# swesterfeld/audiowmark

Measured on AMD Instinct MI355X. Metric: audio seconds watermarked+decoded per wall-second (xRT), 44.1 kHz stereo, higher is better.
Workload: dtype f32; 1 GPU; 60 min stereo 44.1 kHz white noise per GPU resident in HBM, add+get incl. payload decode, payload 0123456789abcdef0011223344556677, strength 10; parallelism=1 GPU, patterns=108, payload_matches=104, ranks_seen=1

## Files before the change

### audiowmark_amd/csrc/hip/viterbi.hip

```cpp
#include "kernels.hh"
#include <atomic>
#include <chrono>
#include <cstdio>
#include <mutex>
#include <type_traits>
#include <utility>

namespace awmk {

namespace {

constexpr int V_ORDER = 15;
constexpr int V_STATES = 1 << V_ORDER;
constexpr int V_WG = 256;

__device__ constexpr unsigned V_GEN_AB[12] = { 066561, 075211, 071545, 054435, 063635, 052475, 063543, 075307, 052547, 045627, 067657, 051757 };

template<int BT> __device__ constexpr unsigned v_gen (int g) { return BT == 2 ? V_GEN_AB[g] : V_GEN_AB[2 * g + BT]; }
__device__ constexpr unsigned v_parity (unsigned v) { v ^= v >> 16; v ^= v >> 8; v ^= v >> 4; v ^= v >> 2; v ^= v >> 1; return v & 1; }

typedef float v2f __attribute__ ((ext_vector_type (2)));

__device__ __forceinline__ v2f
pk_add_sel (v2f d, v2f pair, bool a, bool b)
// ... 240 lines not shown
  float *m_out = reinterpret_cast<float *> (ws + (parity_in ? 0 : V_METRIC_BYTES));
  unsigned int *dec = reinterpret_cast<unsigned int *> (ws + 2 * V_METRIC_BYTES) + dec_offset;
  const float *coded = b.soft[t] + (size_t) blk * b.n_steps * rate;
  const bool finite = *block_flag (ws, b.block_ws_bytes) == 0;
  if (t == 0)
    {
      if (PLAIN && finite) viterbi_round<0, K, true> (coded, step0, m_in, m_out, dec, L);
      else                 viterbi_round<0, K, false> (coded, step0, m_in, m_out, dec, L);
    }
  else if (t == 1)
    {
      if (PLAIN && finite) viterbi_round<1, K, true> (coded, step0, m_in, m_out, dec, L);
      else                 viterbi_round<1, K, false> (coded, step0, m_in, m_out, dec, L);
    }
  else
    {
      if (PLAIN && finite) viterbi_round<2, K, true> (coded, step0, m_in, m_out, dec, L);
      else                 viterbi_round<2, K, false> (coded, step0, m_in, m_out, dec, L);
    }
}

constexpr int SUPER_LDS = 16 * 324;

template<int BT, int NPF, bool COH = false> __device__ __forceinline__ void
viterbi_super_round (const float *coded, int step0, const float *m_in, float *m_out, unsigned int *dec, const size_t (&dec_off)[3],
                     int g, int lane, float *lds_a, float *lds_b, bool in_perm, bool out_perm, bool first = false)
{
  float m[16];
  const int L1 = (lane << 3) | g;
#pragma unroll
  for (int j = 0; j < 16; j++)
    m[j] = first ? ((L1 | j) == 0 ? 0.f : -1.f)
                 : ld_metric<COH> (in_perm ? m_in + g * 4096 + ((j << 8) | lane) : m_in + L1 + j * 2048);
  const int hi = lane >> 4, lo = lane & 15;
#pragma unroll
  for (int r = 0; r < 3; r++)
    {
      const int L = r == 0 ? L1 : r == 1 ? ((hi << 7) | (g << 4) | lo) : ((g << 8) | lane);
      unsigned int words[4];
      if (r < NPF)
        viterbi_steps<BT, 4, false> (coded, step0 + 4 * r, m, words, L);
      else
        viterbi_steps<BT, 4, true> (coded, step0 + 4 * r, m, words, L);
      st_words<COH> (dec + dec_off[r] + (size_t) L * 4, words[0], words[1], words[2], words[3]);
      if (r < 2)
        {
          float *x = r == 0 ? lds_a : lds_b;
#pragma unroll
          for (int loc = 0; loc < 16; loc++)
            x[loc * 324 + lo * 20 + hi] = m[loc];
          __syncthreads();
          const float4 *src = reinterpret_cast<const float4 *> (x + lo * 324 + hi * 20);
#pragma unroll
          for (int q = 0; q < 4; q++)
            {
              const float4 v = src[q];
              m[4 * q] = v.x; m[4 * q + 1] = v.y; m[4 * q + 2] = v.z; m[4 * q + 3] = v.w;
            }
        }
    }
  if (out_perm)
    {
#pragma unroll
      for (int f = 0; f < 8; f++)
        st_pair<COH> (m_out + f * 4096 + (g << 9) + (lane << 1), m[f], m[f + 8]);
      return;
    }
  float *out = m_out + (size_t) ((g << 8) | lane) * 16;
#pragma unroll
  for (int q = 0; q < 4; q++)
    st_quad<COH> (out + 4 * q, m[4 * q], m[4 * q + 1], m[4 * q + 2], m[4 * q + 3]);
}

struct SuperOffsets { size_t off[3]; int in_perm, out_perm, first; };

template<int NPF> __global__ void __launch_bounds__ (V_WG)
viterbi_super_kernel (ViterbiBatch b, int step0, int parity_in, SuperOffsets so)
{
  __shared__ float lds_a[SUPER_LDS], lds_b[SUPER_LDS];
  int blk = blockIdx.y, t = 0;
  if (blk >= b.n[0]) { blk -= b.n[0]; t = 1; }
  if (t == 1 && blk >= b.n[1]) { blk -= b.n[1]; t = 2; }
  const int rate = t == 2 ? 12 : 6;
  const int g = blockIdx.x, lane = threadIdx.x;
  unsigned char *ws = b.ws[t] + (size_t) blk * b.block_ws_bytes;
  const float *m_in = reinterpret_cast<const float *> (ws + (parity_in ? V_METRIC_BYTES : 0));
  float *m_out = reinterpret_cast<float *> (ws + (parity_in ? 0 : V_METRIC_BYTES));
  unsigned int *dec = reinterpret_cast<unsigned int *> (ws + 2 * V_METRIC_BYTES);
  const float *coded = b.soft[t] + (size_t) blk * b.n_steps * rate;
  if (so.first && g == 0)
    {
      const bool has_nan = block_has_nan (coded, b.n_steps * rate);
      if (lane == 0)
        *block_flag (ws, b.block_ws_bytes) = has_nan;
    }
  const bool finite = so.first || *block_flag (ws, b.block_ws_bytes) == 0;
  if (t == 0)
    {
      if (finite) viterbi_super_round<0, NPF> (coded, step0, m_in, m_out, dec, so.off, g, lane, lds_a, lds_b, so.in_perm != 0, so.out_perm != 0, so.first != 0);
      else        viterbi_super_round<0, 3> (coded, step0, m_in, m_out, dec, so.off, g, lane, lds_a, lds_b, so.in_perm != 0, so.out_perm != 0, so.first != 0);
    }
  else if (t == 1)
    {
      if (finite) viterbi_super_round<1, NPF> (coded, step0, m_in, m_out, dec, so.off, g, lane, lds_a, lds_b, so.in_perm != 0, so.out_perm != 0, so.first != 0);
      else        viterbi_super_round<1, 3> (coded, step0, m_in, m_out, dec, so.off, g, lane, lds_a, lds_b, so.in_perm != 0, so.out_perm != 0, so.first != 0);
    }
  else
    {
      if (finite) viterbi_super_round<2, NPF> (coded, step0, m_in, m_out, dec, so.off, g, lane, lds_a, lds_b, so.in_perm != 0, so.out_perm != 0, so.first != 0);
      else        viterbi_super_round<2, 3> (coded, step0, m_in, m_out, dec, so.off, g, lane, lds_a, lds_b, so.in_perm != 0, so.out_perm != 0, so.first != 0);
    }
}

__global__ void __launch_bounds__ (256)
viterbi_init_kernel (ViterbiBatch b)
{
  int blk = blockIdx.y, t = 0;
  if (blk >= b.n[0]) { blk -= b.n[0]; t = 1; }
  if (t == 1 && blk >= b.n[1]) { blk -= b.n[1]; t = 2; }
  unsigned char *ws = b.ws[t] + (size_t) blk * b.block_ws_bytes;
  float *m = reinterpret_cast<float *> (ws);
  const int i = blockIdx.x * 256 + threadIdx.x;
  m[i] = i == 0 ? 0.f : -1.f;
  if (blockIdx.x == 0)
    {
      const int rate = t == 2 ? 12 : 6;
      const bool has_nan = block_has_nan (b.soft[t] + (size_t) blk * b.n_steps * rate, b.n_steps * rate);
      if (threadIdx.x == 0)
        *block_flag (ws, b.block_ws_bytes) = has_nan;
    }
}

constexpr int MAX_ROUNDS = 64;
struct TracePlan
// ... 17 lines not shown
      const int K = plan.k[r];
      const unsigned L = state >> K;
      unsigned loc = state & ((1u << K) - 1);
      const int DW = dec_words (K);
      unsigned int w[5] = { 0, 0, 0, 0, 0 };
      const unsigned int *p = dec + plan.dec_offset[r] + (size_t) L * DW;
      const uint4 a = ld_words<COH> (p);
      w[0] = a.x; w[1] = a.y; w[2] = a.z; w[3] = a.w;
      if (DW == 8)
        w[4] = ld_words<COH> (p + 4).x;
      for (int i = K; i >= 1; i--)
        {
          const int step = plan.step0[r] + i - 1;
          if (step < n_steps - V_ORDER)
            bits[step] = loc & 1;
          const unsigned choose_high = (w[i - 1] >> loc) & 1;
          loc = (loc >> 1) | (choose_high << (K - 1));
        }
      state = L + (loc << (V_ORDER - K));
    }
}

template<bool COH> __device__ __forceinline__ void
viterbi_trace_wave (const TracePlan& plan, int final_parity, const unsigned char *ws, int n_steps, int rate, int *bits, float *error, int lane)
{
  const float *metric = reinterpret_cast<const float *> (ws + (final_parity ? V_METRIC_BYTES : 0));
  const unsigned int *dec = reinterpret_cast<const unsigned int *> (ws + 2 * V_METRIC_BYTES);
  if (lane == 0)
    *error = ld_metric<COH> (metric) / float (n_steps * rate);
  const int n_out = n_steps - V_ORDER;
  auto walk = [&] (const unsigned int (&w)[4], int K, unsigned loc, int step0) -> unsigned {
#pragma unroll
    for (int i = 4; i >= 1; i--)
      if (i <= K)
        {
          const int step = step0 + i - 1;
          if (step < n_out && lane == 0)
            bits[step] = loc & 1;
          const unsigned choose_high = (w[i - 1] >> loc) & 1;
          loc = (loc >> 1) | (choose_high << (K - 1));
        }
    return loc;
  };
  auto pick = [] (const uint4& v, unsigned from_lane, unsigned int (&w)[4]) {
    w[0] = __builtin_amdgcn_readlane (v.x, from_lane);
    w[1] = __builtin_amdgcn_readlane (v.y, from_lane);
    w[2] = __builtin_amdgcn_readlane (v.z, from_lane);
    w[3] = __builtin_amdgcn_readlane (v.w, from_lane);
  };
  unsigned state = 0;
  int r = plan.n_rounds - 1;
  while (r >= 0)
    {
      const int K = plan.k[r];
      if (r >= 2 && K == 4 && plan.k[r - 1] == 4 && plan.k[r - 2] == 4)
        {
          const unsigned L0 = state >> 4;
          const uint4 a = ld_words<COH> (dec + plan.dec_offset[r] + (size_t) L0 * 4);
          const unsigned c1 = lane & 15;
          const uint4 b1 = ld_words<COH> (dec + plan.dec_offset[r - 1] + (size_t) ((L0 >> 4) | (c1 << 7)) * 4);
          uint4 c2[4];
#pragma unroll
          for (int q = 0; q < 4; q++)
            {
              const unsigned idx = lane + 64 * q, c = idx & 15, e = idx >> 4;
              c2[q] = ld_words<COH> (dec + plan.dec_offset[r - 2] + (size_t) ((L0 >> 8) | (c << 3) | (e << 7)) * 4);
            }
          unsigned int w[4];
          pick (a, 0, w);
          const unsigned la = __builtin_amdgcn_readfirstlane (walk (w, 4, state & 15, plan.step0[r]));
          const unsigned s1 = L0 | (la << 11);
          pick (b1, la, w);
          const unsigned lb = __builtin_amdgcn_readfirstlane (walk (w, 4, s1 & 15, plan.step0[r - 1]));
// ... 18 lines not shown
      const unsigned L = state >> K;
      const uint4 a = ld_words<COH> (dec + plan.dec_offset[r] + (size_t) L * dec_words (K));
      unsigned int w[4];
      pick (a, 0, w);
      const unsigned l = __builtin_amdgcn_readfirstlane (walk (w, K, state & ((1u << K) - 1), plan.step0[r]));
      state = L | (l << (V_ORDER - K));
      r--;
    }
}

__global__ void __launch_bounds__ (64)
viterbi_trace_kernel (ViterbiBatch b, TracePlan plan)
{
  const int total = b.n[0] + b.n[1] + b.n[2];
  int blk = blockIdx.x * 64 + threadIdx.x, t = 0;
  if (blk >= total)
    return;
  if (blk >= b.n[0]) { blk -= b.n[0]; t = 1; }
  if (t == 1 && blk >= b.n[1]) { blk -= b.n[1]; t = 2; }
  viterbi_trace_one (plan, plan.final_parity, b.ws[t] + (size_t) blk * b.block_ws_bytes, b.n_steps, t == 2 ? 12 : 6,
                     b.bits[t] + (size_t) blk * (b.n_steps - V_ORDER), &b.error[t][blk]);
}

constexpr int SYNC_STRIDE = 16;

__device__ __forceinline__ void
decode_barrier (unsigned int *counter, unsigned int target, unsigned int *fail, bool wait = true)
{
  asm volatile ("s_waitcnt vmcnt(0)" ::: "memory");
  __syncthreads();
  if (threadIdx.x == 0)
    __hip_atomic_fetch_add (counter, 1u, __ATOMIC_RELAXED, __HIP_MEMORY_SCOPE_AGENT);
  if (!wait)
    return;
  if (threadIdx.x == 0)
    {
      const unsigned long long t0 = __builtin_amdgcn_s_memrealtime();
      while (__hip_atomic_load (counter, __ATOMIC_RELAXED, __HIP_MEMORY_SCOPE_AGENT) < target)
        {
          __builtin_amdgcn_s_sleep (2);
          if (__builtin_amdgcn_s_memrealtime() - t0 > 200000000ull || __hip_atomic_load (fail, __ATOMIC_RELAXED, __HIP_MEMORY_SCOPE_AGENT))
            {
              __hip_atomic_store (fail, 1u, __ATOMIC_RELAXED, __HIP_MEMORY_SCOPE_AGENT);
              break;
            }
        }
    }
  __syncthreads();
}

template<int BT> __device__ __forceinline__ void
viterbi_persistent_decode (const ViterbiBatch& b, const TracePlan& plan, int n_super, int blk, int g, int lane, unsigned int *counter,
                           unsigned int *fail, float *lds_a, float *lds_b)
{
  constexpr int t = BT, rate = BT == 2 ? 12 : 6;
  unsigned char *ws = b.ws[t] + (size_t) blk * b.block_ws_bytes;
  float *metric[2] = { reinterpret_cast<float *> (ws), reinterpret_cast<float *> (ws + V_METRIC_BYTES) };
  unsigned int *dec = reinterpret_cast<unsigned int *> (ws + 2 * V_METRIC_BYTES);
  const float *coded = b.soft[t] + (size_t) blk * b.n_steps * rate;
  const bool finite = !block_has_nan (coded, b.n_steps * rate);
  int parity = 0;
  unsigned int meetings = 0;
  if (n_super == 0)
    {
      for (int i = g * 4096 + 2 * lane; i < (g + 1) * 4096; i += 2 * V_WG)
        st_pair<true> (metric[0] + i, i == 0 ? 0.f : -1.f, -1.f);
      decode_barrier (counter, 8 * ++meetings, fail);
    }
  for (int s = 0; s < n_super; s++)
    {
      const int r = 3 * s, step0 = plan.step0[r];
      const size_t off[3] = { plan.dec_offset[r], plan.dec_offset[r + 1], plan.dec_offset[r + 2] };
      int npf = 0;
      for (int q = 0; q < 3; q++)
        npf += plan.step0[r + q] < V_ORDER;
      if (!finite)
        npf = 3;
      const float *m_in = metric[parity];
      float *m_out = metric[parity ^ 1];
      const bool in_perm = s > 0, out_perm = s + 1 < n_super, first = s == 0;
      if (npf == 0)      viterbi_super_round<BT, 0, true> (coded, step0, m_in, m_out, dec, off, g, lane, lds_a, lds_b, in_perm, out_perm, first);
      else if (npf == 1) viterbi_super_round<BT, 1, true> (coded, step0, m_in, m_out, dec, off, g, lane, lds_a, lds_b, in_perm, out_perm, first);
      else if (npf == 2) viterbi_super_round<BT, 2, true> (coded, step0, m_in, m_out, dec, off, g, lane, lds_a, lds_b, in_perm, out_perm, first);
      else               viterbi_super_round<BT, 3, true> (coded, step0, m_in, m_out, dec, off, g, lane, lds_a, lds_b, in_perm, out_perm, first);
      parity ^= 1;
      decode_barrier (counter, 8 * ++meetings, fail, g == 0 || r + 3 < plan.n_rounds);
    }
  for (int r = 3 * n_super; r < plan.n_rounds; r++)
    {
      const int k = plan.k[r], step0 = plan.step0[r];
      const bool plain = step0 >= V_ORDER && finite;
      const float *m_in = metric[parity];
      float *m_out = metric[parity ^ 1];
      unsigned int *d = dec + plan.dec_offset[r];
      for (int L = g * V_WG + lane; L < (V_STATES >> k); L += 8 * V_WG)
        {
          if (k == 4 && plain)  viterbi_round<BT, 4, true, true> (coded, step0, m_in, m_out, d, L);
          else if (k == 4)      viterbi_round<BT, 4, false, true> (coded, step0, m_in, m_out, d, L);
          else if (plain)       viterbi_round<BT, 3, true, true> (coded, step0, m_in, m_out, d, L);
          else                  viterbi_round<BT, 3, false, true> (coded, step0, m_in, m_out, d, L);
        }
      parity ^= 1;
      decode_barrier (counter, 8 * ++meetings, fail, g == 0 || r + 1 < plan.n_rounds);
    }
  if (g == 0 && lane < 64)
    {
      if (lane == 0)
        __hip_atomic_store (counter, 0u, __ATOMIC_RELAXED, __HIP_MEMORY_SCOPE_AGENT);
      float err = 0.f;
      bool wide = true;
      for (int r = 0; r < plan.n_rounds; r++)
        wide = wide && plan.k[r] <= 4;
      if (wide)
        viterbi_trace_wave<true> (plan, parity, ws, b.n_steps, rate, b.bits[t] + (size_t) blk * (b.n_steps - V_ORDER), &err, lane);
      else if (lane == 0)
        viterbi_trace_one<true> (plan, parity, ws, b.n_steps, rate, b.bits[t] + (size_t) blk * (b.n_steps - V_ORDER), &err);
      if (lane == 0)
        b.error[t][blk] = __hip_atomic_load (fail, __ATOMIC_RELAXED, __HIP_MEMORY_SCOPE_AGENT) ? -2.f : err;
    }
}

template<int K, bool PLAIN> __global__ void __launch_bounds__ (V_WG)
viterbi_last_round_kernel (ViterbiBatch b, int step0, int parity_in, size_t dec_offset, TracePlan plan, unsigned int *sync)
{
  __shared__ int is_last;
  int blk = blockIdx.y, t = 0;
  if (blk >= b.n[0]) { blk -= b.n[0]; t = 1; }
  if (t == 1 && blk >= b.n[1]) { blk -= b.n[1]; t = 2; }
  const int rate = t == 2 ? 12 : 6;
  const int L = blockIdx.x * V_WG + threadIdx.x;
  unsigned char *ws = b.ws[t] + (size_t) blk * b.block_ws_bytes;
  const float *m_in = reinterpret_cast<const float *> (ws + (parity_in ? V_METRIC_BYTES : 0));
  float *m_out = reinterpret_cast<float *> (ws + (parity_in ? 0 : V_METRIC_BYTES));
  unsigned int *dec = reinterpret_cast<unsigned int *> (ws + 2 * V_METRIC_BYTES) + dec_offset;
  const float *coded = b.soft[t] + (size_t) blk * b.n_steps * rate;
  const bool finite = *block_flag (ws, b.block_ws_bytes) == 0;
  if (t == 0)
    {
      if (PLAIN && finite) viterbi_round<0, K, true, true> (coded, step0, m_in, m_out, dec, L);
      else                 viterbi_round<0, K, false, true> (coded, step0, m_in, m_out, dec, L);
    }
  else if (t == 1)
    {
      if (PLAIN && finite) viterbi_round<1, K, true, true> (coded, step0, m_in, m_out, dec, L);
      else                 viterbi_round<1, K, false, true> (coded, step0, m_in, m_out, dec, L);
    }
  else
    {
      if (PLAIN && finite) viterbi_round<2, K, true, true> (coded, step0, m_in, m_out, dec, L);
      else                 viterbi_round<2, K, false, true> (coded, step0, m_in, m_out, dec, L);
    }
  asm volatile ("s_waitcnt vmcnt(0)" ::: "memory");
  __syncthreads();
  unsigned int *counter = sync + SYNC_STRIDE * (1 + blockIdx.y);
  if (threadIdx.x == 0)
    is_last = __hip_atomic_fetch_add (counter, 1u, __ATOMIC_RELAXED, __HIP_MEMORY_SCOPE_AGENT) + 1 == gridDim.x;
  __syncthreads();
  if (is_last && threadIdx.x < 64)
    {
      if (threadIdx.x == 0)
        __hip_atomic_store (counter, 0u, __ATOMIC_RELAXED, __HIP_MEMORY_SCOPE_AGENT);
      float err = 0.f;
      viterbi_trace_wave<true> (plan, plan.final_parity, ws, b.n_steps, rate, b.bits[t] + (size_t) blk * (b.n_steps - V_ORDER), &err, threadIdx.x);
      if (threadIdx.x == 0)
        b.error[t][blk] = err;
    }
}

__global__ void __launch_bounds__ (V_WG)
viterbi_persistent_kernel (ViterbiBatch b, TracePlan plan, int n_super, unsigned int *sync)
{
  __shared__ float lds_a[SUPER_LDS], lds_b[SUPER_LDS];
  __shared__ unsigned int my_ticket;
  const int lane = threadIdx.x;
  if (lane == 0)
    my_ticket = __hip_atomic_fetch_add (&sync[0], 1u, __ATOMIC_RELAXED, __HIP_MEMORY_SCOPE_AGENT);
  __syncthreads();
  const unsigned int ticket = my_ticket;
  const int decode = int (ticket >> 3), g = int (ticket & 7);
  int blk = decode, t = 0;
  if (blk >= b.n[0]) { blk -= b.n[0]; t = 1; }
  if (t == 1 && blk >= b.n[1]) { blk -= b.n[1]; t = 2; }
  unsigned int *counter = sync + SYNC_STRIDE * (1 + decode), *fail = sync + 2;
  if (t == 0)      viterbi_persistent_decode<0> (b, plan, n_super, blk, g, lane, counter, fail, lds_a, lds_b);
  else if (t == 1) viterbi_persistent_decode<1> (b, plan, n_super, blk, g, lane, counter, fail, lds_a, lds_b);
  else             viterbi_persistent_decode<2> (b, plan, n_super, blk, g, lane, counter, fail, lds_a, lds_b);
  __syncthreads();
  if (lane == 0)
    {
      const unsigned int left = __hip_atomic_fetch_add (&sync[1], 1u, __ATOMIC_RELAXED, __HIP_MEMORY_SCOPE_AGENT);
      if (left + 1 == gridDim.x)
        {
          __hip_atomic_store (&sync[0], 0u, __ATOMIC_RELAXED, __HIP_MEMORY_SCOPE_AGENT);
          __hip_atomic_store (&sync[1], 0u, __ATOMIC_RELAXED, __HIP_MEMORY_SCOPE_AGENT);
        }
    }
}

constexpr int V_K = 4;

std::vector<RoundPlan>
plan_rounds (int n_steps)
{
  std::vector<RoundPlan> rounds;
  int threes = 0;
  while (threes < V_K && (n_steps - 3 * threes < 0 || (n_steps - 3 * threes) % V_K))
    threes++;
  if (threes == V_K || n_steps - 3 * threes < 0)
    return rounds;
// ... 15 lines not shown

size_t
viterbi_workspace_bytes (long long coded_len, int rate, long long n_blocks)
{
  const auto rounds = plan_rounds (int (coded_len / rate));
  size_t words = 0;
  for (const auto& r : rounds)
    words += size_t (V_STATES >> r.k) * dec_words (r.k);
  const size_t per_block = ((2 * V_METRIC_BYTES + words * sizeof (unsigned int) + 255) & ~size_t (255)) + V_FLAG_BYTES;
  return per_block * size_t (n_blocks);
}

bool
viterbi_steps_supported (long long n_steps)
{
  if (n_steps < V_ORDER || n_steps > 4 * MAX_ROUNDS)
    return false;
  const auto rounds = plan_rounds (int (n_steps));
  return !rounds.empty() && rounds.size() <= size_t (MAX_ROUNDS);
}

int g_viterbi_super = 1;
extern "C" void awm_debug_set_viterbi_super (int on) { g_viterbi_super = on; }
std::atomic<int>    g_viterbi_persistent { -1 };
std::atomic<double> g_dependent_launch_us { -1.0 };
std::mutex          g_probe_mutex;
constexpr double ONE_LAUNCH_ABOVE_US = 9.0;
extern "C" void awm_debug_set_viterbi_persistent (int on) { g_viterbi_persistent.store (on, std::memory_order_relaxed); }
extern "C" double awm_debug_dependent_launch_us (void) { return g_dependent_launch_us.load (std::memory_order_relaxed); }
static bool
use_one_launch()
{
  const int forced = g_viterbi_persistent.load (std::memory_order_relaxed);
  return forced > 0 || (forced < 0 && g_dependent_launch_us.load (std::memory_order_relaxed) > ONE_LAUNCH_ABOVE_US);
}
const char *
viterbi_form_description()
{
  static thread_local char text[160];
  const int forced = g_viterbi_persistent.load (std::memory_order_relaxed);
  snprintf (text, sizeof (text), "viterbi form: %s (%s; dependent launch probe %.1f us, one launch above %.1f us)",
            use_one_launch() ? "one launch per batch" : "launch chain", forced < 0 ? "chosen by the probe" : "forced by awm_debug_set_viterbi_persistent",
            g_dependent_launch_us.load (std::memory_order_relaxed), ONE_LAUNCH_ABOVE_US);
  return text;
}
extern "C" int awm_debug_viterbi_one_launch_in_use (void) { return use_one_launch() ? 1 : 0; }
// ... 34 lines not shown
}

hipError_t
launch_viterbi (hipStream_t st, const float *const soft[3], const long long n_blocks[3], long long n_steps,
                unsigned char *const decisions_ws[3], int *const bits_out[3], float *const error_out[3], unsigned int *sync_ws)
{
  const long long total = n_blocks[0] + n_blocks[1] + n_blocks[2];
  if (total <= 0)
    return hipSuccess;
  const auto rounds = plan_rounds (int (n_steps));
  if (rounds.empty() || rounds.size() > MAX_ROUNDS || total > 65535)
    return hipErrorInvalidValue;
  ViterbiBatch b;
  for (int i = 0; i < 3; i++)
    {
      b.soft[i] = soft[i];
      b.ws[i] = decisions_ws[i];
      b.bits[i] = bits_out[i];
      b.error[i] = error_out[i];
      b.n[i] = int (n_blocks[i]);
    }
  b.n_steps = int (n_steps);
  b.block_ws_bytes = viterbi_workspace_bytes (n_steps * 6, 6, 1);
  TracePlan tp {};
  tp.n_rounds = int (rounds.size());
  for (size_t r = 0; r < rounds.size(); r++)
    {
      tp.k[r] = (unsigned char) rounds[r].k;
      tp.step0[r] = rounds[r].step0;
      tp.dec_offset[r] = (unsigned int) rounds[r].dec_offset;
    }
  if (sync_ws && use_one_launch())
    {
      int n_super = 0;
      while (V_K == 4 && 3 * n_super + 2 < int (rounds.size()) && rounds[3 * n_super].k == 4 && rounds[3 * n_super + 1].k == 4 && rounds[3 * n_super + 2].k == 4)
        n_super++;
      hipLaunchKernelGGL (viterbi_persistent_kernel, dim3 (8u * (unsigned) total), dim3 (V_WG), 0, st, b, tp, n_super, sync_ws);
      return hipGetLastError();
    }
  const bool fold_init = g_viterbi_super && V_K == 4 && rounds.size() >= 3 && rounds[0].k == V_K && rounds[1].k == V_K && rounds[2].k == V_K;
  if (!fold_init)
    hipLaunchKernelGGL (viterbi_init_kernel, dim3 (V_STATES / 256, (unsigned) total), dim3 (256), 0, st, b);
  int parity = 0;
  for (size_t r = 0; r < rounds.size(); )
    {
      const RoundPlan& rp = rounds[r];
      if (g_viterbi_super && r + 2 < rounds.size() && rounds[r].k == V_K && rounds[r + 1].k == V_K && rounds[r + 2].k == V_K && V_K == 4)
        {
          int npf = 0;
          for (int q = 0; q < 3; q++)
            npf += rounds[r + q].step0 < V_ORDER;
          const bool next_is_super = r + 5 < rounds.size() && rounds[r + 3].k == V_K && rounds[r + 4].k == V_K && rounds[r + 5].k == V_K;
          const SuperOffsets so { { rounds[r].dec_offset, rounds[r + 1].dec_offset, rounds[r + 2].dec_offset }, r > 0, next_is_super, r == 0 && fold_init };
          const dim3 grid (8, (unsigned) total);
          if (npf == 0)
            hipLaunchKernelGGL ((viterbi_super_kernel<0>), grid, dim3 (V_WG), 0, st, b, rp.step0, parity, so);
          else if (npf == 1)
            hipLaunchKernelGGL ((viterbi_super_kernel<1>), grid, dim3 (V_WG), 0, st, b, rp.step0, parity, so);
          else if (npf == 2)
            hipLaunchKernelGGL ((viterbi_super_kernel<2>), grid, dim3 (V_WG), 0, st, b, rp.step0, parity, so);
          else
            hipLaunchKernelGGL ((viterbi_super_kernel<3>), grid, dim3 (V_WG), 0, st, b, rp.step0, parity, so);
          parity ^= 1;
          r += 3;
          continue;
        }
      const bool plain = rp.step0 >= V_ORDER;
      const dim3 grid ((V_STATES >> rp.k) / V_WG, (unsigned) total);
      if (sync_ws && r + 1 == rounds.size() && rp.k <= 4)
        {
          tp.final_parity = parity ^ 1;
          if (rp.k == V_K && plain)
            hipLaunchKernelGGL ((viterbi_last_round_kernel<V_K, true>), grid, dim3 (V_WG), 0, st, b, rp.step0, parity, rp.dec_offset, tp, sync_ws);
          else if (rp.k == V_K)
            hipLaunchKernelGGL ((viterbi_last_round_kernel<V_K, false>), grid, dim3 (V_WG), 0, st, b, rp.step0, parity, rp.dec_offset, tp, sync_ws);
          else if (plain)
            hipLaunchKernelGGL ((viterbi_last_round_kernel<3, true>), grid, dim3 (V_WG), 0, st, b, rp.step0, parity, rp.dec_offset, tp, sync_ws);
          else
            hipLaunchKernelGGL ((viterbi_last_round_kernel<3, false>), grid, dim3 (V_WG), 0, st, b, rp.step0, parity, rp.dec_offset, tp, sync_ws);
          return hipGetLastError();
        }
      if (rp.k == V_K && plain)
        hipLaunchKernelGGL ((viterbi_round_kernel<V_K, true>), grid, dim3 (V_WG), 0, st, b, rp.step0, parity, rp.dec_offset);
      else if (rp.k == V_K)
        hipLaunchKernelGGL ((viterbi_round_kernel<V_K, false>), grid, dim3 (V_WG), 0, st, b, rp.step0, parity, rp.dec_offset);
      else if (plain)
        hipLaunchKernelGGL ((viterbi_round_kernel<3, true>), grid, dim3 (V_WG), 0, st, b, rp.step0, parity, rp.dec_offset);
      else
        hipLaunchKernelGGL ((viterbi_round_kernel<3, false>), grid, dim3 (V_WG), 0, st, b, rp.step0, parity, rp.dec_offset);
      parity ^= 1;
      r++;
    }
  tp.final_parity = parity;
  hipLaunchKernelGGL (viterbi_trace_kernel, dim3 ((unsigned) ((total + 63) / 64)), dim3 (64), 0, st, b, tp);
  return hipGetLastError();
}

}
```

### include/awm_hip.h

```cpp
#ifndef AWM_HIP_H
#define AWM_HIP_H

#include <stddef.h>
#include <stdint.h>

#ifdef __cplusplus
extern "C" {
#endif

#define AWM_ERR_GENERIC    (-1)
#define AWM_ERR_NO_DEVICE  (-2)
#define AWM_ERR_ARG        (-3)
#define AWM_ERR_HIP        (-4)
#define AWM_ERR_IO         (-5)

#define AWM_FRAME_SIZE      1024
#define AWM_N_BANDS         81
#define AWM_BLOCK_FRAMES    2226
#define AWM_SOFT_BITS       858

typedef struct awm_ctx awm_ctx;

const char *awm_last_error (void);
const char *awm_version (void);
// ... 200 lines not shown
int awm_ctx_set_helpers (awm_ctx *ctx, awm_ctx *const *helpers, int n_helpers);

void awm_set_speed_params (int detect_speed, int detect_speed_patient, double try_speed, double test_speed);
size_t awm_resample_ratio_frames (size_t n_frames, int n_channels, int rate, double ratio, double max_in_seconds);
int awm_resample_ratio_d (awm_ctx *ctx, const float *pcm_in_d, size_t n_frames, int n_channels, int rate, double ratio,
                          double max_in_seconds, float *out_d, size_t n_out_frames);
int awm_detect_speed_d (awm_ctx *ctx, const uint8_t key[16], const float *pcm_d, size_t n_frames, int n_channels, int rate,
                        int patient, double *speed_out, double *quality_out);
int awm_speed_clip_location_d (awm_ctx *ctx, const uint8_t key[16], const float *pcm_d, size_t n_frames, int n_channels, int rate,
                               double seconds, int candidates, double *location);
int awm_speed_mags_d (awm_ctx *ctx, const uint8_t key[16], const float *pcm_d, size_t n_frames, int n_channels, int rate,
                      double clip_location, double center, double seconds, size_t max_rows, float *out);
int awm_speed_scan_d (awm_ctx *ctx, const uint8_t key[16], const float *pcm_d, size_t n_frames, int n_channels, int rate,
                      double clip_location, double seconds, double step, int n_steps, int n_center_steps,
                      const double *speeds, int n_speeds, size_t max_out, double *out_speed, double *out_quality);

int    awm_speed_select_n_best (double *speed, double *quality, int count, int n);
double awm_speed_smooth_best (const double *speed, const double *quality, int count, double step, double distance);
size_t awm_speed_clip_positions (const uint8_t key[16], size_t n_values, size_t max_out, uint64_t *positions);
int    awm_speed_clip_candidates (const uint8_t key[16], const float *hashed_values, size_t n, int candidates, double *locations);

void awm_debug_set_viterbi_super (int on);
void awm_debug_set_viterbi_persistent (int on);
double awm_debug_dependent_launch_us (void);
int  awm_debug_viterbi_one_launch_in_use (void);
void awm_debug_set_sliding3 (int on);
void awm_debug_set_refine_form (int form);
int  awm_debug_refine_form (void);
void awm_debug_set_k4s_ablate (int flags);
int  awm_debug_sync_db_sliding_d (awm_ctx *ctx, const float *pcm_d, size_t n_frames, int n_channels, const long long *base_d, size_t n_streams,
                                  int count, int ld, float *out_d);
int  awm_debug_sync_db_sliding_rows_d (awm_ctx *ctx, const float *pcm_d, size_t n_frames, int n_channels, const long long *base_d, const int *count_d,
                                       size_t n_streams, int count0, int rows_per_plane, const int *row_perm_d, const unsigned char *band_pos_d,
                                       long long first, long long last, const long long *stream_range_d, const int *range_index_d, int range_div,
                                       int tables_per_slice, int ld, float *out_d, float *tail_d, long long tail_stream_stride, char *have_d,
                                       long long have_stream_stride);
void awm_debug_set_soft_bits_generic (int on);
void awm_debug_set_scan_generic (int on);
int  awm_debug_scan_generic_launches (void);
void awm_debug_set_chunk_stagger (int mode);
void awm_debug_set_resample_phase (int on);
void awm_debug_set_get_overlap (int on);
void awm_debug_set_speed_compare_wide (int on);
void awm_debug_set_speed_compare_fold (int on);
void awm_debug_set_resample_var_mode (int mode);
void awm_debug_set_speed_overlap (int on);
// ... 62 lines not shown
```

Before: 766,100 xRT.

## Fold Viterbi tail rounds into a shrinking-trellis finish and compute start metrics directly

Replaces the final few full 32768-state Viterbi rounds with an in-LDS tail decode. When the trellis is terminated, the number of live states halves each step, so the tail runs as a shrinking trellis inside the last workgroup and the traceback starts from the resulting state. Optionally (fold mode 2) the first super-round is skipped by computing the reachable-state metrics for the first 12 steps directly, with zeroed decision words. This cuts full-width rounds and kernel launches at the cost of more complex kernels, extra LDS use, and a serial tail step on one workgroup.

```diff
diff --git a/audiowmark_amd/csrc/hip/viterbi.hip b/audiowmark_amd/csrc/hip/viterbi.hip
--- a/audiowmark_amd/csrc/hip/viterbi.hip
+++ b/audiowmark_amd/csrc/hip/viterbi.hip
@@ -286,16 +286,60 @@
 
 constexpr int SUPER_LDS = 16 * 324;
 
-template<int BT, int NPF, bool COH = false> __device__ __forceinline__ void
+template<int BT> __device__ __forceinline__ void
+viterbi_start_metrics (const float *coded, int g, int lane, float (&m)[16])
+{
+  constexpr int rate = BT == 2 ? 12 : 6;
+  const unsigned s0 = (unsigned (lane) << 3) | g, s1 = (unsigned (256 + lane) << 3) | g;
+  float d0 = 0.f, d1 = 0.f;
+#pragma unroll
+  for (int i = 1; i <= 12; i++)
+    {
+      const unsigned a0 = s0 >> (12 - i), a1 = s1 >> (12 - i);
+      float n0 = d0, n1 = d1;
+#pragma unroll
+      for (int p = 0; p < rate; p++)
+        {
+          const float c = coded[(i - 1) * rate + p];
+          const float c1 = __fsub_rn (c, 1.0f);
+          const float e0 = __fmul_rn (c, c), e1 = __fmul_rn (c1, c1);
+          n0 = __fadd_rn (n0, (__popc (a0 & v_gen<BT> (p)) & 1) ? e1 : e0);
+          n1 = __fadd_rn (n1, (__popc (a1 & v_gen<BT> (p)) & 1) ? e1 : e0);
+        }
+      d0 = d0 >= 0.f ? n0 : -1.f;
+      d1 = d1 >= 0.f ? n1 : -1.f;
+    }
+  m[0] = d0;
+  m[1] = d1;
+#pragma unroll
+  for (int j = 2; j < 16; j++)
+    m[j] = -1.f;
+}
+
+constexpr int START_DEC_WORDS = 3 * (V_STATES >> 4) * 4;
+
+template<int BT, int NPF, bool COH = false, bool COH_IN = COH> __device__ __forceinline__ void
 viterbi_super_round (const float *coded, int step0, const float *m_in, float *m_out, unsigned int *dec, const size_t (&dec_off)[3],
-                     int g, int lane, float *lds_a, float *lds_b, bool in_perm, bool out_perm, bool first = false)
+                     int g, int lane, float *lds_a, float *lds_b, bool in_perm, bool out_perm, int first = 0)
 {
   float m[16];
   const int L1 = (lane << 3) | g;
-#pragma unroll
-  for (int j = 0; j < 16; j++)
-    m[j] = first ? ((L1 | j) == 0 ? 0.f : -1.f)
-                 : ld_metric<COH> (in_perm ? m_in + g * 4096 + ((j << 8) | lane) : m_in + L1 + j * 2048);
+  if (first == 2)
+    {
+      unsigned int *z = dec + (size_t) (g * V_WG + lane) * 12;
+      static_assert (START_DEC_WORDS == 8 * V_WG * 12, "eight workgroups zero the first three rounds' decision words");
+#pragma unroll
+      for (int q = 0; q < 3; q++)
+        st_words<COH> (z + 4 * q, 0u, 0u, 0u, 0u);
+      viterbi_start_metrics<BT> (coded, g, lane, m);
+    }
+  else
+    {
+#pragma unroll
+      for (int j = 0; j < 16; j++)
+        m[j] = first ? ((L1 | j) == 0 ? 0.f : -1.f)
+                     : ld_metric<COH_IN> (in_perm ? m_in + g * 4096 + ((j << 8) | lane) : m_in + L1 + j * 2048);
+    }
   const int hi = lane >> 4, lo = lane & 15;
 #pragma unroll
   for (int r = 0; r < 3; r++)
@@ -338,42 +382,60 @@
 
 struct SuperOffsets { size_t off[3]; int in_perm, out_perm, first; };
 
+template<int NPF, bool LAST> __device__ __forceinline__ void
+viterbi_super_body (int t, unsigned char *ws, const float *coded, int coded_len, size_t block_ws_bytes, int step0, int parity_in,
+                    const SuperOffsets& so, float *lds_a, float *lds_b)
+{
+  const int g = blockIdx.x, lane = threadIdx.x;
+  const float *m_in = reinterpret_cast<const float *> (ws + (parity_in ? V_METRIC_BYTES : 0));
+  float *m_out = reinterpret_cast<float *> (ws + (parity_in ? 0 : V_METRIC_BYTES));
+  unsigned int *dec = reinterpret_cast<unsigned int *> (ws + 2 * V_METRIC_BYTES);
+  bool finite = true;
+  if (so.first == 2)
+    {
+      const bool has_nan = block_has_nan (coded, coded_len);
+      if (g == 0 && lane == 0)
+        *block_flag (ws, block_ws_bytes) = has_nan;
+      finite = !has_nan;
+    }
+  else if (so.first)
+    {
+      if (g == 0)
+        {
+          const bool has_nan = block_has_nan (coded, coded_len);
+          if (lane == 0)
+            *block_flag (ws, block_ws_bytes) = has_nan;
+        }
+    }
+  else
+    finite = *block_flag (ws, block_ws_bytes) == 0;
+  if (t == 0)
+    {
+      if (finite) viterbi_super_round<0, NPF, LAST, false> (coded, step0, m_in, m_out, dec, so.off, g, lane, lds_a, lds_b, so.in_perm != 0, so.out_perm != 0, so.first);
+      else        viterbi_super_round<0, 3, LAST, false> (coded, step0, m_in, m_out, dec, so.off, g, lane, lds_a, lds_b, so.in_perm != 0, so.out_perm != 0, so.first);
+    }
+  else if (t == 1)
+    {
+      if (finite) viterbi_super_round<1, NPF, LAST, false> (coded, step0, m_in, m_out, dec, so.off, g, lane, lds_a, lds_b, so.in_perm != 0, so.out_perm != 0, so.first);
+      else        viterbi_super_round<1, 3, LAST, false> (coded, step0, m_in, m_out, dec, so.off, g, lane, lds_a, lds_b, so.in_perm != 0, so.out_perm != 0, so.first);
+    }
+  else
+    {
+      if (finite) viterbi_super_round<2, NPF, LAST, false> (coded, step0, m_in, m_out, dec, so.off, g, lane, lds_a, lds_b, so.in_perm != 0, so.out_perm != 0, so.first);
+      else        viterbi_super_round<2, 3, LAST, false> (coded, step0, m_in, m_out, dec, so.off, g, lane, lds_a, lds_b, so.in_perm != 0, so.out_perm != 0, so.first);
+    }
+}
+
 template<int NPF> __global__ void __launch_bounds__ (V_WG)
 viterbi_super_kernel (ViterbiBatch b, int step0, int parity_in, SuperOffsets so)
 {
-  __shared__ float lds_a[SUPER_LDS], lds_b[SUPER_LDS];
+  __shared__ __attribute__ ((aligned (16))) float lds[2 * SUPER_LDS];
   int blk = blockIdx.y, t = 0;
   if (blk >= b.n[0]) { blk -= b.n[0]; t = 1; }
   if (t == 1 && blk >= b.n[1]) { blk -= b.n[1]; t = 2; }
   const int rate = t == 2 ? 12 : 6;
-  const int g = blockIdx.x, lane = threadIdx.x;
-  unsigned char *ws = b.ws[t] + (size_t) blk * b.block_ws_bytes;
-  const float *m_in = reinterpret_cast<const float *> (ws + (parity_in ? V_METRIC_BYTES : 0));
-  float *m_out = reinterpret_cast<float *> (ws + (parity_in ? 0 : V_METRIC_BYTES));
-  unsigned int *dec = reinterpret_cast<unsigned int *> (ws + 2 * V_METRIC_BYTES);
-  const float *coded = b.soft[t] + (size_t) blk * b.n_steps * rate;
-  if (so.first && g == 0)
-    {
-      const bool has_nan = block_has_nan (coded, b.n_steps * rate);
-      if (lane == 0)
-        *block_flag (ws, b.block_ws_bytes) = has_nan;
-    }
-  const bool finite = so.first || *block_flag (ws, b.block_ws_bytes) == 0;
-  if (t == 0)
-    {
-      if (finite) viterbi_super_round<0, NPF> (coded, step0, m_in, m_out, dec, so.off, g, lane, lds_a, lds_b, so.in_perm != 0, so.out_perm != 0, so.first != 0);
-      else        viterbi_super_round<0, 3> (coded, step0, m_in, m_out, dec, so.off, g, lane, lds_a, lds_b, so.in_perm != 0, so.out_perm != 0, so.first != 0);
-    }
-  else if (t == 1)
-    {
-      if (finite) viterbi_super_round<1, NPF> (coded, step0, m_in, m_out, dec, so.off, g, lane, lds_a, lds_b, so.in_perm != 0, so.out_perm != 0, so.first != 0);
-      else        viterbi_super_round<1, 3> (coded, step0, m_in, m_out, dec, so.off, g, lane, lds_a, lds_b, so.in_perm != 0, so.out_perm != 0, so.first != 0);
-    }
-  else
-    {
-      if (finite) viterbi_super_round<2, NPF> (coded, step0, m_in, m_out, dec, so.off, g, lane, lds_a, lds_b, so.in_perm != 0, so.out_perm != 0, so.first != 0);
-      else        viterbi_super_round<2, 3> (coded, step0, m_in, m_out, dec, so.off, g, lane, lds_a, lds_b, so.in_perm != 0, so.out_perm != 0, so.first != 0);
-    }
+  viterbi_super_body<NPF, false> (t, b.ws[t] + (size_t) blk * b.block_ws_bytes, b.soft[t] + (size_t) blk * b.n_steps * rate, b.n_steps * rate,
+                                  b.block_ws_bytes, step0, parity_in, so, lds, lds + SUPER_LDS);
 }
 
 __global__ void __launch_bounds__ (256)
@@ -437,11 +499,12 @@
 }
 
 template<bool COH> __device__ __forceinline__ void
-viterbi_trace_wave (const TracePlan& plan, int final_parity, const unsigned char *ws, int n_steps, int rate, int *bits, float *error, int lane)
+viterbi_trace_wave (const TracePlan& plan, int final_parity, const unsigned char *ws, int n_steps, int rate, int *bits, float *error, int lane,
+                    unsigned state0 = 0, bool folded_tail = false)
 {
   const float *metric = reinterpret_cast<const float *> (ws + (final_parity ? V_METRIC_BYTES : 0));
   const unsigned int *dec = reinterpret_cast<const unsigned int *> (ws + 2 * V_METRIC_BYTES);
-  if (lane == 0)
+  if (lane == 0 && !folded_tail)
     *error = ld_metric<COH> (metric) / float (n_steps * rate);
   const int n_out = n_steps - V_ORDER;
   auto walk = [&] (const unsigned int (&w)[4], int K, unsigned loc, int step0) -> unsigned {
@@ -463,7 +526,7 @@
     w[2] = __builtin_amdgcn_readlane (v.z, from_lane);
     w[3] = __builtin_amdgcn_readlane (v.w, from_lane);
   };
-  unsigned state = 0;
+  unsigned state = state0;
   int r = plan.n_rounds - 1;
   while (r >= 0)
     {
@@ -528,6 +591,131 @@
                      b.bits[t] + (size_t) blk * (b.n_steps - V_ORDER), &b.error[t][blk]);
 }
 
+constexpr int TAIL_MAX = 14;
+constexpr int TAIL_DEC_WORDS = 264;
+constexpr int TAIL_COST_FLOATS = 2 * TAIL_MAX * 12;
+
+__host__ __device__ constexpr int tail_metric_floats (int T) { return T > 2 ? 1 << (T - 1) : 2; }
+constexpr size_t tail_lds_bytes (int T) { return T > 0 ? (tail_metric_floats (T) + TAIL_COST_FLOATS) * sizeof (float) + TAIL_DEC_WORDS * sizeof (unsigned long long) : 0; }
+
+template<int BT> __device__ __forceinline__ unsigned
+viterbi_tail (const float *coded, int n_steps, int T, const float *metric, float *lds_m, unsigned long long *lds_d, float *lds_c, float *end_metric)
+{
+  constexpr int rate = BT == 2 ? 12 : 6;
+  const int tid = threadIdx.x;
+  if (T == 0)
+    {
+      *end_metric = ld_metric<true> (metric);
+      return 0;
+    }
+  for (int k = tid; k < T * rate; k += V_WG)
+    {
+      const float c = coded[(size_t) (n_steps - T) * rate + k];
+      const float c1 = __fsub_rn (c, 1.0f);
+      lds_c[2 * k] = __fmul_rn (c, c);
+      lds_c[2 * k + 1] = __fmul_rn (c1, c1);
+    }
+  int dbase = 0;
+  for (int i = 0; i < T; i++)
+    {
+      const int half = 1 << (T - 1 - i);
+      const int sh = V_ORDER - T + i + 1;
+      float e0[rate], e1[rate];
+      if (i == 0)
+        {
+          const float *c = coded + (size_t) (n_steps - T) * rate;
+#pragma unroll
+          for (int p = 0; p < rate; p++)
+            {
+              const float c1 = __fsub_rn (c[p], 1.0f);
+              e0[p] = __fmul_rn (c[p], c[p]);
+              e1[p] = __fmul_rn (c1, c1);
+            }
+        }
+      else
+        {
+#pragma unroll
+          for (int p = 0; p < rate; p++)
+            {
+              e0[p] = lds_c[2 * (i * rate + p)];
+              e1[p] = lds_c[2 * (i * rate + p) + 1];
+            }
+        }
+      for (int j0 = 0; j0 < half; j0 += 4 * V_WG)
+        {
+          float old0[4], old1[4];
+#pragma unroll
+          for (int u = 0; u < 4; u++)
+            {
+              const int jc = min (j0 + u * V_WG + tid, half - 1);
+              if (i == 0)
+                {
+                  old0[u] = ld_metric<true> (metric + ((size_t) jc << (sh - 1)));
+                  old1[u] = ld_metric<true> (metric + ((size_t) (jc + half) << (sh - 1)));
+                }
+              else
+                {
+                  old0[u] = lds_m[jc];
+                  old1[u] = lds_m[jc + half];
+                }
+            }
+#pragma unroll
+          for (int u = 0; u < 4; u++)
+            {
+              const int j = j0 + u * V_WG + tid;
+              const unsigned ns = unsigned (j) << sh;
+              float d0 = old0[u], d1 = old1[u];
+#pragma unroll
+              for (int p = 0; p < rate; p++)
+                {
+                  const float term = (__popc (ns & v_gen<BT> (p)) & 1) ? e1[p] : e0[p];
+                  d0 = __fadd_rn (d0, term);
+                  d1 = __fadd_rn (d1, term);
+                }
+              const bool r0 = old0[u] >= 0.f, r1 = old1[u] >= 0.f;
+              const bool high = j < half && (r0 ? (r1 && d1 < d0) : r1);
+              if (j < half)
+                lds_m[j] = high ? d1 : (r0 ? d0 : -1.f);
+              const unsigned long long word = __builtin_amdgcn_ballot_w64 (high);
+              if ((tid & 63) == 0 && j < half)
+                lds_d[dbase + (j >> 6)] = word;
+            }
+        }
+      dbase += half >= 64 ? half >> 6 : 1;
+      __syncthreads();
+    }
+  unsigned j = 0;
+  for (int i = T - 1; i >= 0; i--)
+    {
+      const int half = 1 << (T - 1 - i);
+      dbase -= half >= 64 ? half >> 6 : 1;
+      const unsigned high = unsigned (lds_d[dbase + (j >> 6)] >> (j & 63)) & 1u;
+      j += high * half;
+    }
+  *end_metric = lds_m[0];
+  return j << (V_ORDER - T);
+}
+
+__device__ __forceinline__ void
+viterbi_finish_decode (const TracePlan& plan, int final_parity, int t, const unsigned char *ws, const float *coded, int n_steps, int *bits,
+                       float *error, int tail, float *lds_m, unsigned long long *lds_d, bool failed = false)
+{
+  const int rate = t == 2 ? 12 : 6;
+  const float *metric = reinterpret_cast<const float *> (ws + (final_parity ? V_METRIC_BYTES : 0));
+  float end_metric;
+  unsigned state;
+  if (t == 0)      state = viterbi_tail<0> (coded, n_steps, tail, metric, lds_m, lds_d, reinterpret_cast<float *> (lds_d + TAIL_DEC_WORDS), &end_metric);
+  else if (t == 1) state = viterbi_tail<1> (coded, n_steps, tail, metric, lds_m, lds_d, reinterpret_cast<float *> (lds_d + TAIL_DEC_WORDS), &end_metric);
+  else             state = viterbi_tail<2> (coded, n_steps, tail, metric, lds_m, lds_d, reinterpret_cast<float *> (lds_d + TAIL_DEC_WORDS), &end_metric);
+  if (threadIdx.x < 64)
+    {
+      float unused = 0.f;
+      viterbi_trace_wave<true> (plan, final_parity, ws, n_steps, rate, bits, &unused, threadIdx.x, state, true);
+      if (threadIdx.x == 0)
+        *error = failed ? -2.f : end_metric / float (n_steps * rate);
+    }
+}
+
 constexpr int SYNC_STRIDE = 16;
 
 __device__ __forceinline__ void
@@ -557,7 +745,7 @@
 
 template<int BT> __device__ __forceinline__ void
 viterbi_persistent_decode (const ViterbiBatch& b, const TracePlan& plan, int n_super, int blk, int g, int lane, unsigned int *counter,
-                           unsigned int *fail, float *lds_a, float *lds_b)
+                           unsigned int *fail, float *lds_a, float *lds_b, int skip_first, int tail)
 {
   constexpr int t = BT, rate = BT == 2 ? 12 : 6;
   unsigned char *ws = b.ws[t] + (size_t) blk * b.block_ws_bytes;
@@ -573,7 +761,7 @@
         st_pair<true> (metric[0] + i, i == 0 ? 0.f : -1.f, -1.f);
       decode_barrier (counter, 8 * ++meetings, fail);
     }
-  for (int s = 0; s < n_super; s++)
+  for (int s = skip_first ? 1 : 0; s < n_super; s++)
     {
       const int r = 3 * s, step0 = plan.step0[r];
       const size_t off[3] = { plan.dec_offset[r], plan.dec_offset[r + 1], plan.dec_offset[r + 2] };
@@ -584,7 +772,8 @@
         npf = 3;
       const float *m_in = metric[parity];
       float *m_out = metric[parity ^ 1];
-      const bool in_perm = s > 0, out_perm = s + 1 < n_super, first = s == 0;
+      const bool in_perm = s > 0, out_perm = s + 1 < n_super;
+      const int first = s == 0 ? 1 : (s == 1 && skip_first) ? 2 : 0;
       if (npf == 0)      viterbi_super_round<BT, 0, true> (coded, step0, m_in, m_out, dec, off, g, lane, lds_a, lds_b, in_perm, out_perm, first);
       else if (npf == 1) viterbi_super_round<BT, 1, true> (coded, step0, m_in, m_out, dec, off, g, lane, lds_a, lds_b, in_perm, out_perm, first);
       else if (npf == 2) viterbi_super_round<BT, 2, true> (coded, step0, m_in, m_out, dec, off, g, lane, lds_a, lds_b, in_perm, out_perm, first);
@@ -609,7 +798,15 @@
       parity ^= 1;
       decode_barrier (counter, 8 * ++meetings, fail, g == 0 || r + 1 < plan.n_rounds);
     }
-  if (g == 0 && lane < 64)
+  if (g == 0 && tail >= 0)
+    {
+      if (lane == 0)
+        __hip_atomic_store (counter, 0u, __ATOMIC_RELAXED, __HIP_MEMORY_SCOPE_AGENT);
+      viterbi_finish_decode (plan, parity, t, ws, coded, b.n_steps, b.bits[t] + (size_t) blk * (b.n_steps - V_ORDER), &b.error[t][blk], tail, lds_a,
+                             reinterpret_cast<unsigned long long *> (lds_a + (1 << (TAIL_MAX - 1))),
+                             __hip_atomic_load (fail, __ATOMIC_RELAXED, __HIP_MEMORY_SCOPE_AGENT) != 0);
+    }
+  else if (g == 0 && lane < 64)
     {
       if (lane == 0)
         __hip_atomic_store (counter, 0u, __ATOMIC_RELAXED, __HIP_MEMORY_SCOPE_AGENT);
@@ -627,8 +824,9 @@
 }
 
 template<int K, bool PLAIN> __global__ void __launch_bounds__ (V_WG)
-viterbi_last_round_kernel (ViterbiBatch b, int step0, int parity_in, size_t dec_offset, TracePlan plan, unsigned int *sync)
-{
+viterbi_last_round_kernel (ViterbiBatch b, int step0, int parity_in, size_t dec_offset, TracePlan plan, unsigned int *sync, int tail)
+{
+  extern __shared__ __attribute__ ((aligned (16))) float tail_lds[];
   __shared__ int is_last;
   int blk = blockIdx.y, t = 0;
   if (blk >= b.n[0]) { blk -= b.n[0]; t = 1; }
@@ -662,7 +860,14 @@
   if (threadIdx.x == 0)
     is_last = __hip_atomic_fetch_add (counter, 1u, __ATOMIC_RELAXED, __HIP_MEMORY_SCOPE_AGENT) + 1 == gridDim.x;
   __syncthreads();
-  if (is_last && threadIdx.x < 64)
+  if (is_last && tail > 0)
+    {
+      if (threadIdx.x == 0)
+        __hip_atomic_store (counter, 0u, __ATOMIC_RELAXED, __HIP_MEMORY_SCOPE_AGENT);
+      viterbi_finish_decode (plan, plan.final_parity, t, ws, coded, b.n_steps, b.bits[t] + (size_t) blk * (b.n_steps - V_ORDER), &b.error[t][blk], tail,
+                             tail_lds, reinterpret_cast<unsigned long long *> (tail_lds + tail_metric_floats (tail)));
+    }
+  else if (is_last && threadIdx.x < 64)
     {
       if (threadIdx.x == 0)
         __hip_atomic_store (counter, 0u, __ATOMIC_RELAXED, __HIP_MEMORY_SCOPE_AGENT);
@@ -673,10 +878,38 @@
     }
 }
 
+template<int NPF> __global__ void __launch_bounds__ (V_WG)
+viterbi_super_last_kernel (ViterbiBatch b, int step0, int parity_in, SuperOffsets so, TracePlan plan, unsigned int *sync, int tail)
+{
+  __shared__ __attribute__ ((aligned (16))) float lds[2 * SUPER_LDS];
+  __shared__ int is_last;
+  static_assert (2 * SUPER_LDS >= (1 << (TAIL_MAX - 1)) + 2 * TAIL_DEC_WORDS + TAIL_COST_FLOATS, "the tail's metrics, decisions and costs fit the exchange buffers");
+  int blk = blockIdx.y, t = 0;
+  if (blk >= b.n[0]) { blk -= b.n[0]; t = 1; }
+  if (t == 1 && blk >= b.n[1]) { blk -= b.n[1]; t = 2; }
+  const int rate = t == 2 ? 12 : 6;
+  unsigned char *ws = b.ws[t] + (size_t) blk * b.block_ws_bytes;
+  const float *coded = b.soft[t] + (size_t) blk * b.n_steps * rate;
+  viterbi_super_body<NPF, true> (t, ws, coded, b.n_steps * rate, b.block_ws_bytes, step0, parity_in, so, lds, lds + SUPER_LDS);
+  asm volatile ("s_waitcnt vmcnt(0)" ::: "memory");
+  __syncthreads();
+  unsigned int *counter = sync + SYNC_STRIDE * (1 + blockIdx.y);
+  if (threadIdx.x == 0)
+    is_last = __hip_atomic_fetch_add (counter, 1u, __ATOMIC_RELAXED, __HIP_MEMORY_SCOPE_AGENT) + 1 == gridDim.x;
+  __syncthreads();
+  if (!is_last)
+    return;
+  if (threadIdx.x == 0)
+    __hip_atomic_store (counter, 0u, __ATOMIC_RELAXED, __HIP_MEMORY_SCOPE_AGENT);
+  viterbi_finish_decode (plan, plan.final_parity, t, ws, coded, b.n_steps, b.bits[t] + (size_t) blk * (b.n_steps - V_ORDER), &b.error[t][blk], tail,
+                         lds, reinterpret_cast<unsigned long long *> (lds + (1 << (TAIL_MAX - 1))));
+}
+
 __global__ void __launch_bounds__ (V_WG)
-viterbi_persistent_kernel (ViterbiBatch b, TracePlan plan, int n_super, unsigned int *sync)
-{
-  __shared__ float lds_a[SUPER_LDS], lds_b[SUPER_LDS];
+viterbi_persistent_kernel (ViterbiBatch b, TracePlan plan, int n_super, unsigned int *sync, int skip_first, int tail)
+{
+  __shared__ __attribute__ ((aligned (16))) float lds_a[2 * SUPER_LDS];
+  float *lds_b = lds_a + SUPER_LDS;
   __shared__ unsigned int my_ticket;
   const int lane = threadIdx.x;
   if (lane == 0)
@@ -688,9 +921,9 @@
   if (blk >= b.n[0]) { blk -= b.n[0]; t = 1; }
   if (t == 1 && blk >= b.n[1]) { blk -= b.n[1]; t = 2; }
   unsigned int *counter = sync + SYNC_STRIDE * (1 + decode), *fail = sync + 2;
-  if (t == 0)      viterbi_persistent_decode<0> (b, plan, n_super, blk, g, lane, counter, fail, lds_a, lds_b);
-  else if (t == 1) viterbi_persistent_decode<1> (b, plan, n_super, blk, g, lane, counter, fail, lds_a, lds_b);
-  else             viterbi_persistent_decode<2> (b, plan, n_super, blk, g, lane, counter, fail, lds_a, lds_b);
+  if (t == 0)      viterbi_persistent_decode<0> (b, plan, n_super, blk, g, lane, counter, fail, lds_a, lds_b, skip_first, tail);
+  else if (t == 1) viterbi_persistent_decode<1> (b, plan, n_super, blk, g, lane, counter, fail, lds_a, lds_b, skip_first, tail);
+  else             viterbi_persistent_decode<2> (b, plan, n_super, blk, g, lane, counter, fail, lds_a, lds_b, skip_first, tail);
   __syncthreads();
   if (lane == 0)
     {
@@ -752,6 +985,39 @@
 
 int g_viterbi_super = 1;
 extern "C" void awm_debug_set_viterbi_super (int on) { g_viterbi_super = on; }
+std::atomic<int> g_viterbi_fold { 1 };
+extern "C" void awm_debug_set_viterbi_fold (int mode) { g_viterbi_fold.store (mode < 0 ? 0 : mode > 2 ? 2 : mode, std::memory_order_relaxed); }
+extern "C" int awm_debug_viterbi_fold (void) { return g_viterbi_fold.load (std::memory_order_relaxed); }
+
+namespace {
+
+struct FoldPlan
+{
+  int n_super;
+  int skip_first;
+  int n_run;
+  int tail;
+};
+
+FoldPlan
+plan_folds (const std::vector<RoundPlan>& rounds, int n_steps, bool supers, bool have_sync)
+{
+  FoldPlan fp { 0, 0, int (rounds.size()), -1 };
+  while (supers && V_K == 4 && 3 * fp.n_super + 2 < int (rounds.size()) && rounds[3 * fp.n_super].k == 4 && rounds[3 * fp.n_super + 1].k == 4 && rounds[3 * fp.n_super + 2].k == 4)
+    fp.n_super++;
+  const int fold = g_viterbi_fold.load (std::memory_order_relaxed);
+  if (fold >= 1 && fp.n_super >= 1 && have_sync)
+    {
+      fp.n_run = 3 * fp.n_super;
+      fp.tail = n_steps - 12 * fp.n_super;
+      while (fp.tail > TAIL_MAX)
+        fp.tail -= rounds[fp.n_run++].k;
+    }
+  fp.skip_first = fold >= 2 && fp.n_super >= 2;
+  return fp;
+}
+
+}
 std::atomic<int>    g_viterbi_persistent { -1 };
 std::atomic<double> g_dependent_launch_us { -1.0 };
 std::mutex          g_probe_mutex;
@@ -832,37 +1098,51 @@
     }
   b.n_steps = int (n_steps);
   b.block_ws_bytes = viterbi_workspace_bytes (n_steps * 6, 6, 1);
+  const bool one_launch = sync_ws && use_one_launch();
+  const FoldPlan fp = plan_folds (rounds, int (n_steps), one_launch || g_viterbi_super, sync_ws != nullptr);
   TracePlan tp {};
-  tp.n_rounds = int (rounds.size());
-  for (size_t r = 0; r < rounds.size(); r++)
+  tp.n_rounds = fp.n_run;
+  for (int r = 0; r < fp.n_run; r++)
     {
       tp.k[r] = (unsigned char) rounds[r].k;
       tp.step0[r] = rounds[r].step0;
       tp.dec_offset[r] = (unsigned int) rounds[r].dec_offset;
     }
-  if (sync_ws && use_one_launch())
-    {
-      int n_super = 0;
-      while (V_K == 4 && 3 * n_super + 2 < int (rounds.size()) && rounds[3 * n_super].k == 4 && rounds[3 * n_super + 1].k == 4 && rounds[3 * n_super + 2].k == 4)
-        n_super++;
-      hipLaunchKernelGGL (viterbi_persistent_kernel, dim3 (8u * (unsigned) total), dim3 (V_WG), 0, st, b, tp, n_super, sync_ws);
+  if (one_launch)
+    {
+      hipLaunchKernelGGL (viterbi_persistent_kernel, dim3 (8u * (unsigned) total), dim3 (V_WG), 0, st, b, tp, fp.n_super, sync_ws, fp.skip_first, fp.tail);
       return hipGetLastError();
     }
-  const bool fold_init = g_viterbi_super && V_K == 4 && rounds.size() >= 3 && rounds[0].k == V_K && rounds[1].k == V_K && rounds[2].k == V_K;
+  const bool fold_init = fp.n_super >= 1;
   if (!fold_init)
     hipLaunchKernelGGL (viterbi_init_kernel, dim3 (V_STATES / 256, (unsigned) total), dim3 (256), 0, st, b);
   int parity = 0;
-  for (size_t r = 0; r < rounds.size(); )
+  const size_t n_run = size_t (fp.n_run);
+  for (size_t r = fp.skip_first ? 3 : 0; r < n_run; )
     {
       const RoundPlan& rp = rounds[r];
-      if (g_viterbi_super && r + 2 < rounds.size() && rounds[r].k == V_K && rounds[r + 1].k == V_K && rounds[r + 2].k == V_K && V_K == 4)
+      if (r < size_t (3 * fp.n_super))
         {
           int npf = 0;
           for (int q = 0; q < 3; q++)
             npf += rounds[r + q].step0 < V_ORDER;
-          const bool next_is_super = r + 5 < rounds.size() && rounds[r + 3].k == V_K && rounds[r + 4].k == V_K && rounds[r + 5].k == V_K;
-          const SuperOffsets so { { rounds[r].dec_offset, rounds[r + 1].dec_offset, rounds[r + 2].dec_offset }, r > 0, next_is_super, r == 0 && fold_init };
+          const bool next_is_super = r + 3 < size_t (3 * fp.n_super);
+          const int first = r == 0 ? 1 : (r == 3 && fp.skip_first) ? 2 : 0;
+          const SuperOffsets so { { rounds[r].dec_offset, rounds[r + 1].dec_offset, rounds[r + 2].dec_offset }, r > 0, next_is_super, first };
           const dim3 grid (8, (unsigned) total);
+          if (fp.tail >= 0 && r + 3 == n_run)
+            {
+              tp.final_parity = parity ^ 1;
+              if (npf == 0)
+                hipLaunchKernelGGL ((viterbi_super_last_kernel<0>), grid, dim3 (V_WG), 0, st, b, rp.step0, parity, so, tp, sync_ws, fp.tail);
+              else if (npf == 1)
+                hipLaunchKernelGGL ((viterbi_super_last_kernel<1>), grid, dim3 (V_WG), 0, st, b, rp.step0, parity, so, tp, sync_ws, fp.tail);
+              else if (npf == 2)
+                hipLaunchKernelGGL ((viterbi_super_last_kernel<2>), grid, dim3 (V_WG), 0, st, b, rp.step0, parity, so, tp, sync_ws, fp.tail);
+              else
+                hipLaunchKernelGGL ((viterbi_super_last_kernel<3>), grid, dim3 (V_WG), 0, st, b, rp.step0, parity, so, tp, sync_ws, fp.tail);
+              return hipGetLastError();
+            }
           if (npf == 0)
             hipLaunchKernelGGL ((viterbi_super_kernel<0>), grid, dim3 (V_WG), 0, st, b, rp.step0, parity, so);
           else if (npf == 1)
@@ -877,17 +1157,19 @@
         }
       const bool plain = rp.step0 >= V_ORDER;
       const dim3 grid ((V_STATES >> rp.k) / V_WG, (unsigned) total);
-      if (sync_ws && r + 1 == rounds.size() && rp.k <= 4)
+      if (sync_ws && r + 1 == n_run && rp.k <= 4)
         {
           tp.final_parity = parity ^ 1;
+          const int tail = fp.tail > 0 ? fp.tail : 0;
+          const size_t lds = tail_lds_bytes (tail);
           if (rp.k == V_K && plain)
-            hipLaunchKernelGGL ((viterbi_last_round_kernel<V_K, true>), grid, dim3 (V_WG), 0, st, b, rp.step0, parity, rp.dec_offset, tp, sync_ws);
+            hipLaunchKernelGGL ((viterbi_last_round_kernel<V_K, true>), grid, dim3 (V_WG), lds, st, b, rp.step0, parity, rp.dec_offset, tp, sync_ws, tail);
           else if (rp.k == V_K)
-            hipLaunchKernelGGL ((viterbi_last_round_kernel<V_K, false>), grid, dim3 (V_WG), 0, st, b, rp.step0, parity, rp.dec_offset, tp, sync_ws);
+            hipLaunchKernelGGL ((viterbi_last_round_kernel<V_K, false>), grid, dim3 (V_WG), lds, st, b, rp.step0, parity, rp.dec_offset, tp, sync_ws, tail);
           else if (plain)
-            hipLaunchKernelGGL ((viterbi_last_round_kernel<3, true>), grid, dim3 (V_WG), 0, st, b, rp.step0, parity, rp.dec_offset, tp, sync_ws);
+            hipLaunchKernelGGL ((viterbi_last_round_kernel<3, true>), grid, dim3 (V_WG), lds, st, b, rp.step0, parity, rp.dec_offset, tp, sync_ws, tail);
           else
-            hipLaunchKernelGGL ((viterbi_last_round_kernel<3, false>), grid, dim3 (V_WG), 0, st, b, rp.step0, parity, rp.dec_offset, tp, sync_ws);
+            hipLaunchKernelGGL ((viterbi_last_round_kernel<3, false>), grid, dim3 (V_WG), lds, st, b, rp.step0, parity, rp.dec_offset, tp, sync_ws, tail);
           return hipGetLastError();
         }
       if (rp.k == V_K && plain)
diff --git a/include/awm_hip.h b/include/awm_hip.h
--- a/include/awm_hip.h
+++ b/include/awm_hip.h
@@ -246,6 +246,8 @@
 
 void awm_debug_set_viterbi_super (int on);
 void awm_debug_set_viterbi_persistent (int on);
+void awm_debug_set_viterbi_fold (int mode);
+int  awm_debug_viterbi_fold (void);
 double awm_debug_dependent_launch_us (void);
 int  awm_debug_viterbi_one_launch_in_use (void);
 void awm_debug_set_sliding3 (int on);
```

Result: no change. 760,900 xRT (-0.7%).
